# DeepRec-AI/HybridBackend

Measured on AMD Instinct MI355X. Metric: M-lookups/sec, 26-col Criteo-shape dim16, 1/2/4/8 GPUs; % HBM roofline, higher is better.
Workload: dtype f32

## Files before the change

### hybridbackend_amd/_lib.py

```python
import ctypes as C
import os

_HERE = os.path.dirname(os.path.abspath(__file__))
LIB_PATH = os.environ.get('HBK_LIBRARY') or os.path.join(_HERE, 'lib', 'libhbk_core.so')

INT8, UINT8, INT32, UINT32, INT64, UINT64, HALF, FLOAT, DOUBLE = range(9)
APPLY_SGD, APPLY_ADAGRAD = 0, 2
APPLY_LAZY_ADAM, APPLY_FTRL, APPLY_ROWWISE_ADAGRAD = 3, 4, 5
GRAD_DETERMINISTIC = 1
COMBINER_SUM, COMBINER_MEAN, COMBINER_SQRTN = 0, 1, 2
OK, INVALID_ARGUMENT, UNIMPLEMENTED, INTERNAL = 0, 3, 12, 13
COMM_ID_BYTES = 128


class HbkError(RuntimeError):

  def __init__(self, code, message):
    super().__init__(f'[hbk status {code}] {message}')
    self.code = code


class InvalidArgumentError(HbkError, ValueError):
  pass

# ... 325 lines not shown
    'hbk_comm_rccl_versions': (C.c_int, [vp, vp]),
    'hbk_comm_create': (C.c_int, [vp, vp, i32, i32, i32]),
    'hbk_comm_destroy': (C.c_int, [vp]),
    'hbk_comm_check_async': (C.c_int, [vp]),
    'hbk_comm_world_size': (C.c_int, [vp]),
    'hbk_comm_rank': (C.c_int, [vp]),
    'hbk_comm_stream': (vp, [vp]),
    'hbk_comm_active_ranks': (C.c_int, [vp, i32, vp]),
    'hbk_alltoall_n': (C.c_int, [vp, i32, i32, i32, vp, vp, vp, vp]),
    'hbk_alltoallv_wire_workspace_bytes': (sz, [i32, vp, vp, vp, i32]),
    'hbk_alltoallv_n':
      (C.c_int, [vp, i32, i32, i32, i32, vp, vp, vp, vp, vp, vp, sz, vp]),
    'hbk_allreduce_workspace_bytes': (sz, [i32, vp, i32]),
    'hbk_allreduce_n': (C.c_int, [vp, i32, i32, i32, vp, vp, vp, C.c_float, vp, sz, vp]),
    'hbk_allgatherv': (C.c_int, [vp, i32, vp, vp, vp, vp]),
    'hbk_comm_create_custom': (C.c_int, [vp, vp, i32, i32, i32]),
    'hbk_sharded_layout': (C.c_int, [i32, i32] + [vp] * 12),
    'hbk_sharded_create': (C.c_int, [vp, vp, i32, vp, i32]),
    'hbk_sharded_destroy': (C.c_int, [vp]),
    'hbk_sharded_set_hot_rows': (C.c_int, [vp, vp]),
    'hbk_sharded_set_max_norms': (C.c_int, [vp, vp]),
    'hbk_sharded_set_hash_tables': (C.c_int, [vp, vp]),
    'hbk_sharded_lookup_fwd': (C.c_int, [vp, vp, vp, vp, vp, vp, vp, vp]),
    'hbk_sharded_lookup_fwd_weighted': (C.c_int, [vp, vp, vp, vp, vp, vp, vp, vp, vp]),
    'hbk_sharded_prefetch_on': (C.c_int, [vp, vp, vp, vp]),
    'hbk_sharded_lookup_fwd_begin': (C.c_int, [vp, vp, vp, vp, vp, vp]),
    'hbk_sharded_lookup_fwd_end': (C.c_int, [vp, vp, vp, vp]),
    'hbk_sharded_lookup_fwd_ids': (C.c_int, [vp, vp, vp, vp, vp, vp]),
    'hbk_sharded_lookup_fwd_gather': (C.c_int, [vp, vp]),
    'hbk_sharded_hash_missing': (C.c_int, [vp, vp, vp, vp, vp, vp]),
    'hbk_sharded_prefetch': (C.c_int, [vp, vp, vp, vp]),
    'hbk_sharded_owned_ids': (i64, [vp, i32]),
    'hbk_sharded_last_host_us': (C.c_int, [vp, vp]),
    'hbk_sharded_lookup_bwd': (C.c_int, [vp, vp, vp, C.c_float, vp, vp, vp, vp]),
    'hbk_sharded_lookup_bwd_apply': (C.c_int, [vp, vp, vp, i32, C.c_float, vp, vp, vp, vp]),
    'hbk_sharded_set_adam_slots': (C.c_int, [vp, vp, vp]),
    'hbk_sharded_lookup_bwd_adam': (C.c_int, [vp, vp, vp, vp, C.c_float, vp, vp, vp, vp]),
    'hbk_sharded_set_ftrl_slots': (C.c_int, [vp, vp, vp]),
    'hbk_sharded_lookup_bwd_ftrl': (C.c_int, [vp, vp, vp, vp, C.c_float, vp, vp, vp, vp]),
    'hbk_sharded_set_rowwise_adagrad_slots': (C.c_int, [vp, vp]),
    'hbk_sharded_lookup_bwd_rowwise_adagrad': (C.c_int, [vp, vp, vp, vp, C.c_float, vp, vp, vp, vp]),
    'hbk_sharded_lookup_bwd_weights': (C.c_int, [vp, vp, vp, vp, vp]),
  }
  for name, (res, args) in protos.items():
    fn = getattr(l, name)
    fn.restype = res
    fn.argtypes = args


def lib():
  global _lib
  if _lib is not None:
    return _lib
  if not os.path.exists(LIB_PATH):
    raise ImportError(
      f'{LIB_PATH} not found: the gfx950 HIP extension is not built. '
      'Run `python -c "import __graft_entry__ as g; g.build()"` or '
      '`make -C hybridbackend_amd/csrc`. There is no CPU fallback.')
  import torch
  l = C.CDLL(LIB_PATH, mode=C.RTLD_GLOBAL)
  _declare(l)
  _lib = l
  return l


_testing = None
# ... 142 lines not shown
```

### hybridbackend_amd/csrc/common.h

```cpp
#ifndef HBK_CSRC_COMMON_H_
#define HBK_CSRC_COMMON_H_

#include <hip/hip_runtime.h>
#include <stdarg.h>
#include <stdint.h>
#include <stdio.h>

#include "hbk.h"

namespace hbk {

int fail(int code, const char* fmt, ...);

#define HBK_HIP_OK(expr)                                                         \
  do {                                                                           \
    hipError_t e__ = (expr);                                                     \
    if (e__ != hipSuccess) {                                                     \
      return ::hbk::fail(HBK_INTERNAL, "%s failed: %s (%s:%d)", #expr,           \
                         hipGetErrorString(e__), __FILE__, __LINE__);            \
    }                                                                            \
  } while (0)

#define HBK_REQUIRE(cond, ...)                                                   \
  do {                                                                           \
// ... 94 lines not shown
  int bwd_split_pairs = 0;
  int bwd_onepass = 1;
  int fwd_xcd = 1;
  int bwd_xcd = 1;
  int bwd_wide = 1;
  int bwd_group_cols = 0;
  int bwd_dense = 1;
  int bwd_scatter_staged = 1;
  int bwd_rowsort_pos = 64;
  int bwd_pairs_packed = 1;
  int bwd_seg_inline = 1;
  int bwd_scale_fused = 1;
  int bwd_deterministic = 0;
  int bwd_simple = 1;
  int bwd_streams = 4;
  int bwd_lds_pad = 0;
  int bwd_trace = 0;
  int bwd_large_first = 0;
  int bwd_rowsort_ratio = 8;
  int bwd_weights_lds = 1;
  int fwd_d16 = 1;
  int fwd_interleave = 2;
  int fwd_hot_rows = 0;
  int unique_buckets_log2 = -1;
  int partition_sub_tiles = 1;
  int partition_fixed_max = 8;
  int partition_onepass = 1;
  int unique_onepass = 1;
  int sharded_groups = 0;
  int sharded_id64 = 0;
  int sharded_copy_self = 0;
  int sharded_trace = 0;
  int sharded_pack_early = 1;
  int sharded_wire_fused = 1;
  int sharded_inline = 1;
  int sharded_p2p = 1;
  int sharded_p2p_test_refuse = -1;
  int sync_wait_ms = 2000;
  int sync_onepass_off = 0;
  int sync_test_withhold = -1;
};
Options& options();

struct SyncTake {
  int32_t* words;
  int32_t* zero;
  int64_t zero_words;
  int32_t* status;
  int32_t* summary;
  int32_t* poison;
  unsigned long long wait_ticks;
  int32_t withhold;
};
struct SyncWait {
  int32_t* status;
  int32_t* summary;
  int32_t* poison;
  unsigned long long ticks;
  int32_t withhold;
  int32_t pad_;
};
inline SyncWait sync_wait_of(const SyncTake& t) {
  SyncWait w;
  w.status = t.status;
  w.summary = t.summary;
  w.poison = t.poison;
// ... 89 lines not shown
```

### hybridbackend_amd/csrc/misc.cpp

```cpp
#include <stdlib.h>
#include <string.h>

#include <vector>

#include "common.h"

namespace hbk {
namespace {
thread_local char g_last_error[1024] = "";
}

int fail(int code, const char* fmt, ...) {
  va_list ap;
  va_start(ap, fmt);
  vsnprintf(g_last_error, sizeof(g_last_error), fmt, ap);
  va_end(ap);
  return code;
}
}

namespace hbk {
namespace {
struct OptionEntry {
  const char* name;
// ... 10 lines not shown
    {"bwd_scatter_staged", "HBK_BWD_SCATTER_STAGED", &Options::bwd_scatter_staged},
    {"bwd_rowsort_pos", "HBK_BWD_ROWSORT_POS", &Options::bwd_rowsort_pos},
    {"bwd_rowsort_ratio", "HBK_BWD_ROWSORT_RATIO", &Options::bwd_rowsort_ratio},
    {"bwd_deterministic", "HBK_BWD_DETERMINISTIC", &Options::bwd_deterministic},
    {"bwd_streams", "HBK_BWD_STREAMS", &Options::bwd_streams},
    {"bwd_trace", "HBK_BWD_TRACE", &Options::bwd_trace},
    {"bwd_lds_pad", "HBK_BWD_LDS_PAD", &Options::bwd_lds_pad},
    {"bwd_large_first", "HBK_BWD_LARGE_FIRST", &Options::bwd_large_first},
    {"bwd_pairs_packed", "HBK_BWD_PAIRS_PACKED", &Options::bwd_pairs_packed},
    {"bwd_seg_inline", "HBK_BWD_SEG_INLINE", &Options::bwd_seg_inline},
    {"bwd_scale_fused", "HBK_BWD_SCALE_FUSED", &Options::bwd_scale_fused},
    {"bwd_simple", "HBK_BWD_SIMPLE", &Options::bwd_simple},
    {"fwd_d16", "HBK_FWD_D16", &Options::fwd_d16},
    {"bwd_weights_lds", "HBK_BWD_WEIGHTS_LDS", &Options::bwd_weights_lds},
    {"bwd_wide", "HBK_BWD_WIDE", &Options::bwd_wide},
    {"bwd_xcd", "HBK_BWD_XCD", &Options::bwd_xcd},
    {"fwd_xcd", "HBK_FWD_XCD", &Options::fwd_xcd},
    {"fwd_hot_rows", "HBK_FWD_HOT", &Options::fwd_hot_rows},
    {"fwd_interleave", "HBK_FWD_INTERLEAVE", &Options::fwd_interleave},
    {"unique_buckets_log2", "HBK_UNIQUE_LOG2P", &Options::unique_buckets_log2},
    {"partition_sub_tiles", "HBK_PART_SUB", &Options::partition_sub_tiles},
    {"partition_fixed_max", "HBK_PART_FIXED", &Options::partition_fixed_max},
    {"partition_onepass", "HBK_PART_ONEPASS", &Options::partition_onepass},
    {"unique_onepass", "HBK_UNIQUE_ONEPASS", &Options::unique_onepass},
    {"sharded_groups", "HBK_SHARDED_GROUPS", &Options::sharded_groups},
    {"sharded_id64", "HBK_SHARDED_ID64", &Options::sharded_id64},
    {"sharded_copy_self", "HBK_SHARDED_COPY_SELF", &Options::sharded_copy_self},
    {"sharded_trace", "HBK_SHARDED_TRACE", &Options::sharded_trace},
    {"sharded_inline", "HBK_SHARDED_INLINE", &Options::sharded_inline},
    {"sharded_p2p", "HBK_SHARDED_P2P", &Options::sharded_p2p},
    {"sharded_p2p_test_refuse", "HBK_SHARDED_P2P_TEST_REFUSE", &Options::sharded_p2p_test_refuse},
    {"sharded_wire_fused", "HBK_SHARDED_WIRE_FUSED", &Options::sharded_wire_fused},
    {"sharded_pack_early", "HBK_SHARDED_PACK_EARLY", &Options::sharded_pack_early},
    {"sync_wait_ms", "HBK_SYNC_WAIT_MS", &Options::sync_wait_ms},
    {"sync_onepass_off", "HBK_SYNC_ONEPASS_OFF", &Options::sync_onepass_off},
    {"sync_test_withhold", "HBK_SYNC_TEST_WITHHOLD", &Options::sync_test_withhold},
};

Options from_environment() {
  Options o;
  for (const OptionEntry& e : kOptions) {
    const char* v = getenv(e.env);
    if (v != nullptr && *v != 0) o.*(e.field) = atoi(v);
  }
  return o;
}
}

Options& options() {
  static Options o = from_environment();
  return o;
}
}

extern "C" const char* hbk_last_error(void) { return hbk::g_last_error; }

extern "C" int hbk_set_option(const char* name, int32_t value) {
  using namespace hbk;
  HBK_REQUIRE(name != nullptr, "set_option: name is NULL");
  for (const OptionEntry& e : kOptions) {
    if (strcmp(e.name, name) == 0) {
      options().*(e.field) = value;
      return HBK_OK;
    }
  }
  return fail(HBK_INVALID_ARGUMENT, "set_option: unknown option '%s'", name);
// ... 117 lines not shown
```

### hybridbackend_amd/csrc/sharded.hip

```cpp
#include <stdio.h>
#include <stdlib.h>
#include <string.h>
#include <unistd.h>

#include <algorithm>
#include <chrono>
#include <functional>
#include <random>
#include <utility>
#include <vector>

#include "common.h"

namespace hbk {
int alltoallv_events(hbk_comm_t comm, int32_t n, int32_t dtype, int32_t wire_dtype,
                     int32_t topology, const int64_t* common_sizes, const void* const* inputs,
                     const int32_t* send_sizes, void* const* outputs,
                     const int32_t* recv_sizes, void* wire_ws, size_t wire_ws_bytes,
                     hbk_stream_t compute_stream, hipEvent_t before, hipEvent_t after,
                     bool skip_self, bool inline_x);
int partition_by_modulo_fused(int32_t n_cols, int32_t num_partitions, const int64_t* const* inputs,
                              const int64_t* lens, const int64_t* buckets,
                              int64_t* const* outputs, int32_t* const* sizes,
                              int32_t* const* indices, int32_t* sizes_t, void* workspace,
                              size_t workspace_bytes, hipStream_t stream);
namespace {

constexpr int kBlock = 256;
constexpr int kMaxSegs = 480;
constexpr int kMaxPackWorldP2p = 256;
constexpr int kCopyTileBytes = kBlock * 16 * 8;

struct Seg {
  const void* src;
  void* dst;
  int64_t bytes;
  int32_t tile0;
  int32_t narrow;
};

struct SegArgs {
  int32_t n_segs;
  int32_t pad_;
  Seg seg[kMaxSegs];
};
// ... 195 lines not shown
      } else {
        qh = mid;
      }
    }
    const int64_t at = base[q] + (e - cum[q]);
    if (at < 0 || at >= a.dst_items) continue;
    if (a.narrow) {
      reinterpret_cast<int32_t*>(a.dst)[at] = (int32_t)v;
    } else {
      reinterpret_cast<int64_t*>(a.dst)[at] = v;
    }
  }
  if (a.slots == nullptr) return;
  const int32_t* idx = a.idx[c];
#pragma unroll
  for (int k = 0; k < kPackTile / kBlock; ++k) {
    const int32_t j = e0 + k * kBlock + tid;
    if (j >= n) break;
    const int32_t e = __builtin_nontemporal_load(idx + j);
    if (e < 0 || e >= cum[W]) continue;
    int q = 0, qh = W;
    while (qh - q > 1) {
      const int mid = (q + qh) >> 1;
      if (cum[mid] <= e) {
        q = mid;
      } else {
        qh = mid;
      }
    }
    const int64_t at = base[q] + (e - cum[q]);
    if (at < 0 || at >= a.dst_items) continue;
    a.slots[at] = j;
  }
}

constexpr int kDedupTile = 2048;

struct DedupArgs {
  const int64_t* uniq;
  const int32_t* inv;
  int32_t* idx;
  const int32_t* nu;
  int32_t* S;
  int32_t* St;
  FastDiv wdiv;
  int32_t n_cols, W, N, pad_;
  int64_t off[kMaxPackCols];
  int32_t n[kMaxPackCols];
  int32_t tile0[kMaxPackCols];
  int16_t col[kMaxPackCols];
};
static_assert(sizeof(DedupArgs) <= 16384, "kernarg budget");

__global__ __launch_bounds__(kBlock) void dedup_compose_kernel(const DedupArgs a) {
  int d = 0, hi = a.n_cols;
  while (hi - d > 1) {
    const int mid = (d + hi) >> 1;
    if (a.tile0[mid] <= (int)blockIdx.x) {
      d = mid;
    } else {
      hi = mid;
    }
  }
  const int32_t n = a.n[d];
  const int32_t* inv = a.inv + a.off[d];
  int32_t* idx = a.idx + a.off[d];
// ... 161 lines not shown
  bool trace;
  int n_groups;
  bool inline_x;
  std::vector<hbk_sharded_column_t> cols;
  std::vector<int64_t> n_ids, n_seg;
  std::vector<int64_t> n_sent;
  std::vector<const int32_t*> row_splits;
  hbk::SlotPair adam;
  hbk::SlotPair ftrl;
  hbk::SlotPair rowwise;
  std::vector<float> max_norms;
  std::vector<int32_t> lowp;
  bool lowp_wire16 = false;
  std::vector<hbk_sharded_hash_t> hash;
  bool any_hash = false;
  hbk::Buffer slots_buf;
  std::vector<const float*> id_weights;
  std::vector<int32_t> send_sizes;
  std::vector<int32_t> recv_sizes;
  std::vector<hbk::Group> groups;
  std::vector<int64_t> fwd_own_id_off;
  hipEvent_t ev[4][4];
  bool have_step;
  bool rows_live = false;
  float host_us[3];
  hbk::Buffer part_ws, ids_buf, rows_buf, wire_ws, bwd_ws, runs_dev;
  char* send_ids_p;
  char* recv_ids_p;
  float* send_rows_p;
  float* recv_rows_p;
  bool any_dedup;
  hbk::Buffer dedup_tmp;
  bool pack_early;
  bool fused_half;
  bool zero_copy_grads;
  bool zero_copy_self;
  struct PartSet {
    hbk::Buffer part_out, shard_index, sizes_dev;
    hbk::Buffer uniq, inv, nu, uniq_ws;
    hbk::Buffer packed;
    bool packed_early = false;
    hbk::Buffer slots;
    bool has_slots = false;
    int32_t* host_sizes = nullptr;
    hipEvent_t done = nullptr;
    hipEvent_t ready = nullptr;
    std::vector<const int64_t*> ids;
    std::vector<int64_t> n_ids;
    bool pending = false;
  } ps[2];
  int cur;
  hipStream_t pre_stream;
  hipEvent_t step_begin;
  bool prefetch_used;
  bool fwd_open = false;
  bool ids_open = false;
  bool fin_wire = false, fin_hop = false, fin_p2p = false;
  bool fin_prefetched = false;
  int32_t* fin_slot_send = nullptr;
  hbk::Buffer missing_ws;
  int fin_use = 0;
  std::chrono::steady_clock::time_point fin_t0;
  float fin_us[2] = {0.f, 0.f};
  bool p2p_opt = false;
  bool p2p_bound = false;
  std::vector<float*> p2p_outs;
// ... 12 lines not shown
  HBK_REQUIRE(plan != nullptr && comm != nullptr, "sharded_create: NULL argument");
  HBK_REQUIRE(n_cols >= 1 && cols != nullptr, "sharded_create: need at least one column");
  HBK_REQUIRE(wire_dtype == HBK_FLOAT || wire_dtype == HBK_HALF,
              "sharded_create: wire_dtype must be float or half");
  for (int32_t c = 0; c < n_cols; ++c) {
    HBK_REQUIRE(cols[c].dim >= 1 && cols[c].rows_local >= 0 && cols[c].bucket >= 0,
                "sharded_create: column %d: bad dim / rows / bucket", c);
    HBK_REQUIRE(cols[c].combiner >= HBK_COMBINER_SUM && cols[c].combiner <= HBK_COMBINER_SQRTN,
                "sharded_create: column %d: unknown combiner %d", c, cols[c].combiner);
    HBK_REQUIRE(cols[c].shard != nullptr || cols[c].rows_local == 0,
                "sharded_create: column %d: shard is NULL", c);
  }
  hbk_sharded* p = new hbk_sharded();
  p->comm = comm;
  p->W = hbk_comm_world_size(comm);
  p->rank = hbk_comm_rank(comm);
  p->N = n_cols;
  p->wire_dtype = wire_dtype;
  p->cols.assign(cols, cols + n_cols);
  p->max_norms.assign((size_t)n_cols, 0.0f);
  p->id32 = options().sharded_id64 == 0;
  p->trace = options().sharded_trace != 0;
  p->n_groups = options().sharded_groups;
  p->inline_x = options().sharded_inline != 0;
  p->p2p_opt = options().sharded_p2p != 0;
  for (int32_t c = 0; c < n_cols; ++c) {
    if (cols[c].bucket <= 0 || cols[c].bucket > 0x7fffffffll) p->id32 = false;
  }
  p->have_step = false;
  p->any_dedup = false;
  for (int32_t c = 0; c < n_cols; ++c) p->any_dedup = p->any_dedup || cols[c].dedup != 0;
  p->fused_half = wire_dtype == HBK_HALF && options().sharded_wire_fused != 0;
  p->pack_early = options().sharded_pack_early != 0;
  p->zero_copy_self = (wire_dtype == HBK_FLOAT || p->fused_half) && options().sharded_copy_self == 0;
  p->zero_copy_grads = p->zero_copy_self && wire_dtype == HBK_FLOAT;
  p->send_ids_p = p->recv_ids_p = nullptr;
  p->send_rows_p = p->recv_rows_p = nullptr;
  p->cur = 0;
  p->pre_stream = nullptr;
  p->step_begin = nullptr;
  p->prefetch_used = false;
  p->host_runs = nullptr;
  for (auto& st : p->ev) {
    for (auto& e : st) {
      if (hipEventCreateWithFlags(&e, hipEventDisableTiming) != hipSuccess) {
        delete p;
        return fail(HBK_INTERNAL, "sharded_create: hipEventCreate failed");
      }
    }
  }
  bool ok = hipEventCreateWithFlags(&p->step_begin, hipEventDisableTiming) == hipSuccess;
  for (auto& set : p->ps) {
    ok = ok && hipEventCreateWithFlags(&set.done, hipEventDisableTiming) == hipSuccess &&
         hipEventCreateWithFlags(&set.ready, hipEventDisableTiming) == hipSuccess &&
         hipHostMalloc(reinterpret_cast<void**>(&set.host_sizes),
                       sizeof(int32_t) * 3 * (size_t)n_cols * p->W,
                       hipHostMallocDefault) == hipSuccess;
  }
  if (!ok ||
      hipHostMalloc(reinterpret_cast<void**>(&p->host_runs),
                    sizeof(int64_t) * 7 * (size_t)n_cols * p->W, hipHostMallocDefault) !=
          hipSuccess) {
    hbk_sharded_destroy(p);
    return fail(HBK_INTERNAL, "sharded_create: could not create streams / events / pinned memory");
  }
  *plan = p;
// ... 54 lines not shown
  s.narrow = narrow;
  return s;
}

int exchange(hbk_sharded* p, int32_t dtype, int32_t wire, const void* in, const int32_t* send,
             void* out, const int32_t* recv, hbk_stream_t stream, hipEvent_t before = nullptr,
             hipEvent_t after = nullptr, void* wire_ws = nullptr, size_t wire_ws_bytes = 0,
             bool skip_self = false) {
  const int64_t cs[1] = {1};
  const void* vin[1] = {in};
  void* vout[1] = {out};
  if (wire != dtype && wire_ws == nullptr) {
    const size_t wws = hbk_alltoallv_wire_workspace_bytes(1, cs, send, recv, p->W);
    int rc = p->wire_ws.ensure(wws + 16);
    if (rc != HBK_OK) return rc;
    wire_ws = p->wire_ws.ptr;
    wire_ws_bytes = p->wire_ws.bytes;
  }
  return alltoallv_events(p->comm, 1, dtype, wire, HBK_TOPOLOGY_ALL, cs, vin, send, vout, recv,
                          wire_ws, wire_ws_bytes, stream, before, after, skip_self,
                          p->inline_x && before != nullptr);
}

int pipeline_groups(int n_cols, int world, int requested) {
  int g = requested >= 1 && requested <= 4 ? requested : 2;
  if (world == 1 && !(requested >= 1 && requested <= 4)) g = 1;
  return g < n_cols ? g : n_cols;
}

int step_groups(const hbk_sharded* p) {
  if (p->p2p_bound) return 1;
  return p->inline_x && !(p->n_groups >= 1 && p->n_groups <= 4)
             ? 1 : pipeline_groups(p->N, p->W, p->n_groups);
}

int run_partition(hbk_sharded* p, hbk_sharded::PartSet& set, const int64_t* const* ids,
                  const int64_t* n_ids, hipStream_t stream) {
  const int N = p->N, W = p->W;
  int64_t total = 0;
  for (int c = 0; c < N; ++c) {
    HBK_REQUIRE(n_ids[c] >= 0 && n_ids[c] < (1ll << 31), "sharded lookup: bad n_ids[%d]", c);
    total += n_ids[c];
  }
  int rc;
  if ((rc = set.part_out.ensure((size_t)total * 8 + 8)) != HBK_OK) return rc;
  if ((rc = set.shard_index.ensure((size_t)total * 4 + 8)) != HBK_OK) return rc;
  if ((rc = set.sizes_dev.ensure((size_t)N * W * 4 * 3)) != HBK_OK) return rc;
  if ((rc = set.packed.ensure((size_t)total * (p->id32 ? 4 : 8) + 16)) != HBK_OK) return rc;
  std::vector<int64_t*> pout(N);
  std::vector<int32_t*> sizes(N), idx(N);
  std::vector<int64_t> buckets(N);
  int32_t* sizes_dev = reinterpret_cast<int32_t*>(set.sizes_dev.ptr);
  int32_t* sizes_t = sizes_dev + (size_t)N * W;
  int32_t* recv_t = sizes_t + (size_t)N * W;
  int64_t off = 0;
  for (int c = 0; c < N; ++c) {
    pout[c] = reinterpret_cast<int64_t*>(set.part_out.ptr) + off;
    idx[c] = reinterpret_cast<int32_t*>(set.shard_index.ptr) + off;
    sizes[c] = sizes_dev + (size_t)c * W;
    buckets[c] = p->cols[c].bucket;
    off += n_ids[c];
  }
  const size_t ws = hbk_partition_workspace_bytes(N, n_ids, W);
  if ((rc = p->part_ws.ensure(ws + 8)) != HBK_OK) return rc;
  rc = partition_by_modulo_fused(N, W, ids, n_ids, buckets.data(), pout.data(), sizes.data(),
                                 idx.data(), sizes_t, p->part_ws.ptr, p->part_ws.bytes, stream);
// ... 40 lines not shown
                        set.uniq_ws.ptr, set.uniq_ws.bytes, reinterpret_cast<hbk_stream_t>(stream));
      if (rc != HBK_OK) return rc;
      a.uniq = reinterpret_cast<const int64_t*>(set.uniq.ptr);
      a.inv = reinterpret_cast<const int32_t*>(set.inv.ptr);
      a.idx = reinterpret_cast<int32_t*>(set.shard_index.ptr);
      a.nu = reinterpret_cast<const int32_t*>(set.nu.ptr);
      a.S = sizes_dev;
      a.St = sizes_t;
      a.wdiv = make_fastdiv((uint64_t)W);
      a.wdiv.d = (uint64_t)W;
      a.n_cols = nd;
      a.W = W;
      a.N = N;
      a.pad_ = 0;
      hipLaunchKernelGGL(dedup_compose_kernel, dim3((unsigned)tiles), dim3(kBlock), 0, stream, a);
      hipLaunchKernelGGL(dedup_sizes_kernel, dim3((unsigned)nd), dim3(kMaxPackWorld), 0, stream, a);
      HBK_HIP_OK(hipGetLastError());
    }
  }
  const void* sin[1] = {sizes_t};
  void* sout[1] = {recv_t};
  const int64_t cnt[1] = {(int64_t)N * W};
  rc = hbk_alltoall_n(p->comm, 1, HBK_INT32, HBK_TOPOLOGY_ALL, sin, cnt, sout,
                      reinterpret_cast<hbk_stream_t>(stream));
  if (rc != HBK_OK) return rc;
  HBK_HIP_OK(hipMemcpyAsync(set.host_sizes, sizes_dev, sizeof(int32_t) * 3 * N * W,
                            hipMemcpyDeviceToHost, stream));
  HBK_HIP_OK(hipEventRecord(set.done, stream));
  set.packed_early = p->pack_early && N <= kMaxPackCols && W <= kMaxPackWorld && total > 0;
  set.has_slots = false;
  if (set.packed_early) {
    PackArgs a;
    a.slots = nullptr;
    if (p->p2p_bound) {
      if ((rc = set.slots.ensure((size_t)total * 4 + 16)) != HBK_OK) return rc;
      a.slots = reinterpret_cast<int32_t*>(set.slots.ptr);
      set.has_slots = true;
    }
    a.S = sizes_dev;
    a.dst = set.packed.ptr;
    a.dst_items = total;
    a.n_cols = N;
    a.W = W;
    a.narrow = p->id32 ? 1 : 0;
    a.pad_ = 0;
    const int G = step_groups(p);
    int64_t tiles = 0, gbase = 0;
    for (int g = 0; g < G; ++g) {
      const int c0 = (int)((int64_t)N * g / G), c1 = (int)((int64_t)N * (g + 1) / G);
      int64_t in_group = 0;
      for (int c = c0; c < c1; ++c) {
        a.src[c] = id_src[c];
        a.idx[c] = idx[c];
        a.gbase[c] = gbase;
        a.n[c] = (int32_t)n_ids[c];
        a.tile0[c] = (int32_t)tiles;
        a.g0[c] = (int16_t)c0;
        a.g1[c] = (int16_t)c1;
        tiles += (n_ids[c] + kPackTile - 1) / kPackTile;
        in_group += n_ids[c];
      }
      gbase += in_group;
    }
    hipLaunchKernelGGL(pack_ids_kernel, dim3((unsigned)tiles), dim3(kBlock), 0, stream, a);
    HBK_HIP_OK(hipGetLastError());
  }
  HBK_HIP_OK(hipEventRecord(set.ready, stream));
// ... 577 lines not shown
      }
      c0 += k;
    }
  }
  const bool wire = !(W == 1 && zc);
  const bool hop = wire && !p->inline_x;
  if (hop) HBK_HIP_OK(hipEventRecord(p->ev[0][0], stream));
  for (int g = 0; g < G && wire; ++g) {
    const Group& gr = groups[g];
    rc = exchange(p, id_dtype, id_dtype, ids_send_base + gr.id_send * id_bytes,
                  gr.lay.ids_send_peer.data(), ids_recv_base + gr.id_recv * id_bytes,
                  gr.lay.ids_recv_peer.data(), stream_, p->ev[0][0], p->ev[1][g], nullptr, 0, zc);
    if (rc != HBK_OK) return rc;
    if (p2p) {
      rc = exchange(p, HBK_INT32, HBK_INT32, slot_send + gr.id_send, gr.lay.ids_send_peer.data(),
                    slot_recv + gr.id_recv, gr.lay.ids_recv_peer.data(), stream_, p->ev[0][0],
                    p->ev[3][0], nullptr, 0, zc);
      if (rc != HBK_OK) return rc;
    }
  }
  p->fin_wire = wire;
  p->fin_hop = hop;
  p->fin_p2p = p2p;
  p->fin_use = use;
  p->fin_t0 = t_begin;
  p->fin_us[0] = (float)t_enq1;
  p->fin_us[1] = (float)(t_sync - t_enq1);
  p->fin_prefetched = prefetched;
  p->fin_slot_send = slot_send;
  p->ids_open = true;
  return HBK_OK;
}

int fwd_gather(hbk_sharded_t p, hbk_stream_t stream_) {
  p->ids_open = false;
  hipStream_t stream = as_stream(stream_);
  const int N = p->N, W = p->W, me = p->rank;
  const bool wire = p->fin_wire, hop = p->fin_hop, p2p = p->fin_p2p;
  const bool zc = p->zero_copy_self, half = p->fused_half, any_hash = p->any_hash;
  const bool lowp = !p->lowp.empty(), wire16 = p->lowp_wire16;
  const int32_t id_dtype = p->id32 ? HBK_INT32 : HBK_INT64;
  const std::vector<Group>& groups = p->groups;
  const int G = (int)groups.size();
  int64_t* const slots_base = reinterpret_cast<int64_t*>(p->slots_buf.ptr);
  int32_t* const slot_send = p->fin_slot_send;
  int32_t* const slot_recv = reinterpret_cast<int32_t*>(p->slot_recv.ptr);
  float* const rows_send_base = p->send_rows_p;
  float* const rows_recv_base = p->recv_rows_p;
  int rc;
  for (int g = 0; g < G; ++g) {
    const Group& gr = groups[g];
    const int ng = gr.c1 - gr.c0;
    if (hop) HBK_HIP_OK(hipStreamWaitEvent(stream, p->ev[1][g], 0));
    if (hop && p2p) HBK_HIP_OK(hipStreamWaitEvent(stream, p->ev[3][0], 0));
    auto run_ids = [&](int q, int c) { return received_ids_at(p, gr, q, c); };
    if (any_hash && (rc = translate_group(p, gr, run_ids, slots_base, stream_)) != HBK_OK) return rc;
    std::vector<hbk_lookup_column_t> v;
    std::vector<float> clip;
    std::vector<int32_t> lowp_dtype;
    v.reserve((size_t)ng * W);
    for (int q = 0; q < W; ++q) {
      for (int c = 0; c < ng; ++c) {
        const int64_t n = gr.R[(size_t)q * ng + c];
        if (n == 0) continue;
        clip.push_back(p->max_norms[(size_t)(gr.c0 + c)]);
        if (lowp) lowp_dtype.push_back(p->lowp[(size_t)(gr.c0 + c)]);
        const hbk_sharded_column_t& col = p->cols[gr.c0 + c];
        hbk_lookup_column_t h;
        memset(&h, 0, sizeof(h));
        h.table = col.shard;
        h.rows = col.rows_local;
        h.dim = col.dim;
        h.ids_dtype = id_dtype;
        h.n_ids = n;
        h.n_segments = n;
        h.divisor = W;
        h.combiner = HBK_COMBINER_SUM;
        h.hot_rows = col.hot_rows;
        int64_t out_at = gr.row_send + gr.lay.own_row_off[(size_t)q * ng + c];
        float* out_base = rows_send_base;
        h.ids = run_ids(q, c);
        if (any_hash && p->hash[(size_t)(gr.c0 + c)].keys_cache != nullptr) {
          h.ids_dtype = HBK_INT64;
          h.ids = slots_base + gr.id_recv + gr.lay.own_id_off[(size_t)q * ng + c];
          h.divisor = 1;
        }
        if (zc && q == me) {
          out_at = gr.row_recv + gr.lay.req_row_off[(size_t)q * ng + c];
          out_base = rows_recv_base;
        }
        if (p2p) {
          h.out = p->peer_out[(size_t)q * N + gr.c0 + c];
          h.out_stride = p->peer_stride[(size_t)q * N + gr.c0 + c];
          h.out_slots = slot_recv + gr.id_recv + gr.lay.own_id_off[(size_t)q * ng + c];
          if (zc && q == me) {
            h.out_slots = slot_send + gr.id_send + gr.lay.req_id_off[(size_t)q * ng + c];
          }
          h.hot_rows = 0;
        } else if (half || wire16) {
          h.out = reinterpret_cast<float*>(reinterpret_cast<uint16_t*>(out_base) + out_at);
          h.half_io = half ? HBK_LOOKUP_OUT_HALF : 0;
        } else {
          h.out = out_base + out_at;
        }
        v.push_back(h);
      }
    }
    if (lowp) {
      if (wire16) {
        std::vector<hbk_lowp_gather_column_t> lv(v.size());
        for (size_t i = 0; i < v.size(); ++i) {
          const hbk_lookup_column_t& h = v[i];
          hbk_lowp_gather_column_t& d = lv[i];
          memset(&d, 0, sizeof(d));
          d.table = h.table;
          d.dim = h.dim;
          d.ids_dtype = h.ids_dtype;
          d.rows = h.rows;
          d.ids = h.ids;
          d.n_ids = h.n_ids;
          d.divisor = h.divisor;
          d.out = h.out;
        }
        rc = hbk_lowp_gather_rows_n((int32_t)lv.size(), lv.data(), stream_);
      } else {
        std::vector<hbk_lowp_lookup_column_t> lv(v.size());
        for (size_t i = 0; i < v.size(); ++i) {
          const hbk_lookup_column_t& h = v[i];
          hbk_lowp_lookup_column_t& d = lv[i];
          memset(&d, 0, sizeof(d));
          d.table = h.table;
// ... 159 lines not shown
      HBK_REQUIRE(outs[c] == p->p2p_outs[c] &&
                      (out_strides == nullptr || out_strides[c] == 0 ||
                       out_strides[c] == p->p2p_strides[c] ||
                       (out_strides[c] == p->cols[c].dim && p->p2p_strides[c] == p->cols[c].dim)),
                  "sharded_lookup_fwd: column %d: not the output registered with "
                  "hbk_sharded_p2p_bind", c);
    }
  }
  for (int g = 0; g < G && wire && !p2p; ++g) {
    const Group& gr = groups[g];
    if (half || wire16) {
      rc = exchange(p, HBK_HALF, HBK_HALF, reinterpret_cast<uint16_t*>(rows_send_base) + gr.row_send,
                    gr.lay.rows_send_peer.data(),
                    reinterpret_cast<uint16_t*>(rows_recv_base) + gr.row_recv,
                    gr.lay.rows_recv_peer.data(), stream_, p->ev[2][g], p->ev[3][g], nullptr, 0, zc);
    } else {
      rc = exchange(p, HBK_FLOAT, p->wire_dtype, rows_send_base + gr.row_send,
                    gr.lay.rows_send_peer.data(), rows_recv_base + gr.row_recv,
                    gr.lay.rows_recv_peer.data(), stream_, p->ev[2][g], p->ev[3][g],
                    p->wire_ws.ptr, p->wire_ws.bytes, zc);
    }
    if (rc != HBK_OK) return rc;
  }
  std::vector<int32_t*> idx((size_t)N);
  {
    int64_t off = 0;
    for (int c = 0; c < N; ++c) {
      idx[c] = reinterpret_cast<int32_t*>(set.shard_index.ptr) + off;
      off += n_ids[c];
    }
  }
  const int64_t* d_start = reinterpret_cast<const int64_t*>(p->runs_dev.ptr);
  const int64_t* d_base = d_start + (size_t)N * W;
  for (int g = 0; g < G && !p2p; ++g) {
    const Group& gr = groups[g];
    const int ng = gr.c1 - gr.c0;
    if (hop) HBK_HIP_OK(hipStreamWaitEvent(stream, p->ev[3][g], 0));
    std::vector<hbk_lookup_column_t> v(ng);
    for (int c = 0; c < ng; ++c) {
      const int cc = gr.c0 + c;
      hbk_lookup_column_t& h = v[c];
      memset(&h, 0, sizeof(h));
      h.table = half || wire16 ? reinterpret_cast<const float*>(reinterpret_cast<const uint16_t*>(rows_recv_base) +
                                                                gr.row_recv)
                               : rows_recv_base + gr.row_recv;
      h.half_io = half ? HBK_LOOKUP_TABLE_HALF : 0;
      h.rows = p->n_sent[cc];
      h.dim = p->cols[cc].dim;
      h.ids_dtype = HBK_INT32;
      h.ids = idx[cc];
      h.n_ids = n_ids[cc];
      h.row_splits = p->row_splits[cc];
      h.n_segments = p->n_seg[cc];
      h.divisor = 1;
      h.combiner = p->cols[cc].combiner;
      h.out = outs[cc];
      h.out_stride = out_strides ? out_strides[cc] : 0;
      h.run_start = d_start + (size_t)cc * W;
      h.run_base = d_base + (size_t)cc * W;
      h.n_runs = W;
      h.id_weights = p->id_weights[cc];
    }
    if (wire16) {
      std::vector<hbk_lowp_lookup_runs_column_t> lv((size_t)ng);
      for (int c = 0; c < ng; ++c) {
        const hbk_lookup_column_t& h = v[c];
        hbk_lowp_lookup_runs_column_t& d = lv[(size_t)c];
        memset(&d, 0, sizeof(d));
        d.col.table = h.table;
        d.col.table_dtype = p->lowp[(size_t)(gr.c0 + c)];
        d.col.dim = h.dim;
        d.col.rows = h.rows;
        d.col.ids = h.ids;
        d.col.ids_dtype = h.ids_dtype;
        d.col.combiner = h.combiner;
        d.col.n_ids = h.n_ids;
        d.col.row_splits = h.row_splits;
        d.col.n_segments = h.n_segments;
        d.col.divisor = 1;
        d.col.out_stride = h.out_stride;
        d.col.out = h.out;
        d.col.id_weights = h.id_weights;
        d.run_start = h.run_start;
        d.run_base = h.run_base;
        d.n_runs = h.n_runs;
      }
      rc = hbk_lowp_lookup_fwd_runs(ng, lv.data(), stream_);
    } else {
      rc = hbk_group_lookup_fwd(ng, v.data(), stream_);
    }
    if (rc != HBK_OK) return rc;
  }
  p->have_step = true;
  p->rows_live = !p2p;
  const double total = std::chrono::duration<double, std::micro>(std::chrono::steady_clock::now() -
                                                                p->fin_t0).count();
  p->host_us[0] = p->fin_us[0];
  p->host_us[1] = p->fin_us[1];
  p->host_us[2] = (float)(total - p->fin_us[0] - p->fin_us[1]);
  return HBK_OK;
}

extern "C" int hbk_sharded_lookup_fwd(hbk_sharded_t p, const int64_t* const* ids,
                                      const int64_t* n_ids,
                                      const int32_t* const* row_splits,
                                      const int64_t* n_segments, float* const* outs,
                                      const int32_t* out_strides, hbk_stream_t stream_) {
  using namespace hbk;
  HBK_REQUIRE(outs != nullptr, "sharded_lookup_fwd: NULL argument array");
  const int rc = hbk_sharded_lookup_fwd_begin(p, ids, n_ids, row_splits, n_segments, stream_);
  if (rc != HBK_OK) return rc;
  return hbk_sharded_lookup_fwd_end(p, outs, out_strides, stream_);
}

extern "C" int hbk_sharded_lookup_fwd_weighted(hbk_sharded_t p, const int64_t* const* ids,
                                               const int64_t* n_ids,
                                               const int32_t* const* row_splits,
                                               const int64_t* n_segments,
                                               const float* const* id_weights, float* const* outs,
                                               const int32_t* out_strides, hbk_stream_t stream_) {
  using namespace hbk;
  HBK_REQUIRE(p != nullptr && outs != nullptr, "sharded_lookup_fwd: NULL argument");
  bool weighted = false;
  for (int c = 0; id_weights != nullptr && c < p->N; ++c) weighted = weighted || id_weights[c] != nullptr;
  for (int c = 0; weighted && c < p->N; ++c) {
    HBK_REQUIRE(id_weights[c] == nullptr || p->cols[c].bucket > 0,
                "sharded_lookup_fwd_weighted: column %d: id_weights need a bucket (hbk_sharded_column_t."
                "bucket > 0) so that every id names a row of its owner's shard", c);
  }
  if (weighted && p->p2p_bound) {
    return fail(HBK_UNIMPLEMENTED, "sharded_lookup_fwd_weighted: the p2p form (hbk_sharded_p2p_bind) has "
                "no stitch to apply id_weights in");
  }
  int rc = hbk_sharded_lookup_fwd_begin(p, ids, n_ids, row_splits, n_segments, stream_);
  if (rc != HBK_OK) return rc;
  for (int c = 0; weighted && c < p->N; ++c) p->id_weights[c] = id_weights[c];
  return hbk_sharded_lookup_fwd_end(p, outs, out_strides, stream_);
}

extern "C" int hbk_sharded_prefetch_on(hbk_sharded_t p, const int64_t* const* ids,
                                       const int64_t* n_ids, hbk_stream_t stream_) {
  using namespace hbk;
  HBK_REQUIRE(p != nullptr && ids && n_ids, "sharded_prefetch_on: NULL argument");
  hbk_sharded::PartSet& set = p->ps[p->cur ^ 1];
// ... 515 lines not shown
    return fail(HBK_UNIMPLEMENTED, "%s: the plan has a hash column (hbk_sharded_set_hash_tables): its rows are fp32",
                who);
  }
  if (p->p2p_bound) {
    return fail(HBK_UNIMPLEMENTED, "%s: the plan is p2p-bound (hbk_sharded_p2p_bind): the p2p form's owner gather "
                "stores fp32 rows", who);
  }
  p->adam = SlotPair();
  p->ftrl = SlotPair();
  p->rowwise = SlotPair();
  p->lowp.assign(dtypes, dtypes + p->N);
  p->lowp_wire16 = wire == HBK_LOWP_WIRE_TABLE;
  p->have_step = false;
  p->rows_live = false;
  p->fwd_open = p->ids_open = false;
  return HBK_OK;
}

extern "C" int hbk_sharded_set_hot_rows(hbk_sharded_t p, const int32_t* hot_rows) {
  using namespace hbk;
  HBK_REQUIRE(p != nullptr && hot_rows != nullptr, "sharded_set_hot_rows: NULL argument");
  for (int c = 0; c < p->N; ++c) p->cols[c].hot_rows = hot_rows[c] != 0 ? 1 : 0;
  return HBK_OK;
}

extern "C" int hbk_sharded_last_host_us(hbk_sharded_t p, float* out3) {
  using namespace hbk;
  HBK_REQUIRE(p != nullptr && out3 != nullptr, "sharded_last_host_us: NULL argument");
  HBK_REQUIRE(p->have_step, "sharded_last_host_us: no forward step yet");
  for (int i = 0; i < 3; ++i) out3[i] = p->host_us[i];
  return HBK_OK;
}

extern "C" int64_t hbk_sharded_owned_ids(hbk_sharded_t p, int32_t column) {
  if (p == nullptr || !(p->have_step || p->ids_open || p->fwd_open) || column < 0 || column >= p->N) return -1;
  int64_t n = 0;
  for (int q = 0; q < p->W; ++q) n += p->recv_sizes[(size_t)q * p->N + column];
  return n;
}
```

### hybridbackend_amd/embedding/sharded.py

```python
import ctypes as C
import threading

import torch

from hybridbackend_amd import _lib
from hybridbackend_amd import _marshal
from hybridbackend_amd.distribute import partition as _partition
from hybridbackend_amd.embedding.lookup import GroupLookup
from hybridbackend_amd.embedding.lookup import GroupLookupGrad
from hybridbackend_amd.embedding import optimizer as _opt


class _Step:
  __slots__ = ('ids', 'row_splits', 'send_ids', 'send_sizes', 'shard_index', 'send_sizes_host',
               'recv_sizes_host', 'recv_ids', 'send_rows', 'recv_rows', 'outs')

  def __init__(self):
    for s in self.__slots__:
      setattr(self, s, None)


_PLAN_LOCK = threading.RLock()


# ... 84 lines not shown
    from hybridbackend_amd.embedding.lookup import _combiner_code
    n = len(self.shards)
    combs = self.combiners
    if isinstance(combs, (str, int)) or combs is None:
      combs = [combs] * n
    cols = (_lib.ShardedColumn * n)()
    for c, t in enumerate(self.shards):
      cols[c].shard = t.data_ptr()
      cols[c].rows_local = t.shape[0]
      cols[c].dim = t.shape[1]
      cols[c].combiner = _combiner_code(combs[c])
      cols[c].bucket = self.buckets[c]
      cols[c].hot_rows = 1 if self.hot_rows[c] else 0
      cols[c].dedup = 1 if self.dedup[c] else 0
      if self.accums is not None:
        cols[c].accum = self.accums[c].data_ptr()
    self._plan_handle = C.c_void_p()
    wire = _lib.HALF if self.wire_dtype == torch.float16 else _lib.FLOAT
    _lib.check(self._lib.hbk_sharded_create(
      C.byref(self._plan_handle), self.coll._handle, n, cols, wire))
    self._plan_created()
    if any(self.max_norms):
      _lib.check(self._lib.hbk_sharded_set_max_norms(self._plan_handle, (C.c_float * n)(*self.max_norms)))
    for opt, slots in _opt.bound(self):
      opt.set_sharded_slots(self._plan_handle, slots)

  def _plan_created(self):
    """Hook: plan state a subclass sets right after creation (ShardedHashGroupLookup: its tables)."""

  def last_host_us(self):
    out = (C.c_float * 3)()
    _lib.check(self._lib.hbk_sharded_last_host_us(self._plan(), out))
    return tuple(float(v) for v in out)

  def p2p_bind(self, outs):
    n = len(self.shards)
    if len(outs) != n:
      raise _lib.InvalidArgumentError(_lib.INVALID_ARGUMENT, f'p2p_bind: {len(outs)} outputs for {n} columns')
    for c, o in enumerate(outs):
      _lib.require_device_tensor(o, 'output', row_strided=True)
      if o.dtype != torch.float32 or o.dim() != 2 or o.shape[1] != self.dims[c]:
        raise _lib.InvalidArgumentError(_lib.INVALID_ARGUMENT, f'p2p_bind: output {c} must be fp32 [*, {self.dims[c]}]')
    strides = (C.c_int32 * n)(*[0 if o.is_contiguous() else int(o.stride(0)) for o in outs])
    rows = _lib.i64_array([int(o.shape[0]) for o in outs])
    rc = self._lib.hbk_sharded_p2p_bind(self._plan(), _lib.ptr_array([o.data_ptr() for o in outs]),
                                        strides, rows, _lib.current_stream(self.device))
    if rc == _lib.UNIMPLEMENTED:
      self._p2p_keep = None
      return False
    _lib.check(rc)
    self._p2p_keep = list(outs)
    return True

  def p2p_unbind(self):
    _lib.check(self._lib.hbk_sharded_p2p_unbind(self._plan()))
    self._p2p_keep = None

  def close(self):
    if getattr(self, '_plan_handle', None) is not None:
      self._lib.hbk_sharded_destroy(self._plan_handle)
      self._plan_handle = None

  def bind(self, ids, row_splits=None, outs=None, sp_weights=None):
    bound = self._bind(ids, row_splits, outs)
    if sp_weights is not None and any(w is not None for w in sp_weights):
      from hybridbackend_amd import _marshal
# ... 391 lines not shown
```

### include/hbk.h

```cpp
#ifndef HBK_H_
#define HBK_H_

#include <stddef.h>
#include <stdint.h>

#ifdef __cplusplus
extern "C" {
#endif

typedef void* hbk_stream_t;

#define HBK_OK 0
#define HBK_INVALID_ARGUMENT 3
#define HBK_UNIMPLEMENTED 12
#define HBK_INTERNAL 13

#define HBK_INT8 0
#define HBK_UINT8 1
#define HBK_INT32 2
#define HBK_UINT32 3
#define HBK_INT64 4
#define HBK_UINT64 5
#define HBK_HALF 6
#define HBK_FLOAT 7
// ... 678 lines not shown
} hbk_sharded_hash_t;
int hbk_sharded_set_hash_tables(hbk_sharded_t plan, const hbk_sharded_hash_t* tables );
int hbk_sharded_destroy(hbk_sharded_t plan);
int hbk_sharded_lookup_fwd(hbk_sharded_t plan, const int64_t* const* ids, const int64_t* n_ids,
                           const int32_t* const* row_splits, const int64_t* n_segments,
                           float* const* outs, const int32_t* out_strides, hbk_stream_t stream);
int hbk_sharded_lookup_fwd_weighted(hbk_sharded_t plan, const int64_t* const* ids,
                                    const int64_t* n_ids, const int32_t* const* row_splits,
                                    const int64_t* n_segments, const float* const* id_weights,
                                    float* const* outs, const int32_t* out_strides,
                                    hbk_stream_t stream);
int hbk_sharded_lookup_fwd_begin(hbk_sharded_t plan, const int64_t* const* ids,
                                 const int64_t* n_ids, const int32_t* const* row_splits,
                                 const int64_t* n_segments, hbk_stream_t stream);
int hbk_sharded_lookup_fwd_end(hbk_sharded_t plan, float* const* outs, const int32_t* out_strides,
                               hbk_stream_t stream);
int hbk_sharded_lookup_fwd_ids(hbk_sharded_t plan, const int64_t* const* ids, const int64_t* n_ids,
                               const int32_t* const* row_splits, const int64_t* n_segments,
                               hbk_stream_t stream);
int hbk_sharded_lookup_fwd_gather(hbk_sharded_t plan, hbk_stream_t stream);
int hbk_sharded_hash_missing(hbk_sharded_t plan, const uint8_t* want , int64_t* const* out_ids,
                             const int64_t* out_capacity, int64_t* counts ,
                             hbk_stream_t stream);
int hbk_sharded_prefetch(hbk_sharded_t plan, const int64_t* const* ids, const int64_t* n_ids,
                         void* ids_ready_event );
int hbk_sharded_prefetch_on(hbk_sharded_t plan, const int64_t* const* ids, const int64_t* n_ids,
                            hbk_stream_t stream);
int64_t hbk_sharded_owned_ids(hbk_sharded_t plan, int32_t column);

int hbk_sharded_p2p_bind(hbk_sharded_t plan, float* const* outs, const int32_t* out_strides,
                         const int64_t* out_rows, hbk_stream_t stream);
int hbk_sharded_p2p_unbind(hbk_sharded_t plan);
int hbk_sharded_last_host_us(hbk_sharded_t plan, float* out3);
int hbk_sharded_lookup_bwd_weights(hbk_sharded_t plan, const float* const* grads,
                                   const int32_t* grad_strides, float* const* grad_weights,
                                   hbk_stream_t stream);
int hbk_sharded_lookup_bwd(hbk_sharded_t plan, const float* const* grads,
                           const int32_t* grad_strides, float apply_lr,
                           int64_t* const* unique_rows, float* const* grad_rows,
                           int32_t* const* n_unique, hbk_stream_t stream);
int hbk_sharded_lookup_bwd_apply(hbk_sharded_t plan, const float* const* grads,
                                 const int32_t* grad_strides, int32_t apply, float apply_lr,
                                 int64_t* const* unique_rows, float* const* grad_rows,
                                 int32_t* const* n_unique, hbk_stream_t stream);
int hbk_sharded_set_adam_slots(hbk_sharded_t plan, float* const* m, float* const* v);
int hbk_sharded_lookup_bwd_adam(hbk_sharded_t plan, const float* const* grads,
                                const int32_t* grad_strides, const hbk_adam_t* adam, float lr,
                                int64_t* const* unique_rows, float* const* grad_rows,
                                int32_t* const* n_unique, hbk_stream_t stream);
int hbk_sharded_set_ftrl_slots(hbk_sharded_t plan, float* const* accum, float* const* linear);
int hbk_sharded_lookup_bwd_ftrl(hbk_sharded_t plan, const float* const* grads,
                                const int32_t* grad_strides, const hbk_ftrl_t* ftrl, float lr,
                                int64_t* const* unique_rows, float* const* grad_rows,
                                int32_t* const* n_unique, hbk_stream_t stream);
int hbk_sharded_set_rowwise_adagrad_slots(hbk_sharded_t plan, float* const* accum);
int hbk_sharded_lookup_bwd_rowwise_adagrad(hbk_sharded_t plan, const float* const* grads,
                                           const int32_t* grad_strides,
                                           const hbk_rowwise_adagrad_t* rowwise_adagrad, float lr,
                                           int64_t* const* unique_rows, float* const* grad_rows,
                                           int32_t* const* n_unique, hbk_stream_t stream);

#ifdef __cplusplus
}
#endif
#endif
```

Before: 29970.

## Write local lookups directly to outputs and scatter received rows by slot

For simple float-wire sharded forward lookups at small world sizes, the local shard writes gathered rows straight into the caller's output tensors using the pack slot map. It skips the intermediate receive buffer and the reassembly pass. Rows received from peers go through a new multi-run scatter kernel that places them at their slot positions, replacing the per-column run-based gather. This removes one round of HBM traffic for self-owned rows, at the cost of writing slots during packing, extra host-side eligibility checks, and a new kernel launch path.

```diff
diff --git a/hybridbackend_amd/_lib.py b/hybridbackend_amd/_lib.py
--- a/hybridbackend_amd/_lib.py
+++ b/hybridbackend_amd/_lib.py
@@ -381,6 +381,7 @@
     'hbk_sharded_prefetch': (C.c_int, [vp, vp, vp, vp]),
     'hbk_sharded_owned_ids': (i64, [vp, i32]),
     'hbk_sharded_last_host_us': (C.c_int, [vp, vp]),
+    'hbk_sharded_last_form': (C.c_int, [vp, vp]),
     'hbk_sharded_lookup_bwd': (C.c_int, [vp, vp, vp, C.c_float, vp, vp, vp, vp]),
     'hbk_sharded_lookup_bwd_apply': (C.c_int, [vp, vp, vp, i32, C.c_float, vp, vp, vp, vp]),
     'hbk_sharded_set_adam_slots': (C.c_int, [vp, vp, vp]),
diff --git a/hybridbackend_amd/csrc/common.h b/hybridbackend_amd/csrc/common.h
--- a/hybridbackend_amd/csrc/common.h
+++ b/hybridbackend_amd/csrc/common.h
@@ -150,6 +150,7 @@
   int sharded_copy_self = 0;
   int sharded_trace = 0;
   int sharded_pack_early = 1;
+  int sharded_direct = 1;
   int sharded_wire_fused = 1;
   int sharded_inline = 1;
   int sharded_p2p = 1;
diff --git a/hybridbackend_amd/csrc/misc.cpp b/hybridbackend_amd/csrc/misc.cpp
--- a/hybridbackend_amd/csrc/misc.cpp
+++ b/hybridbackend_amd/csrc/misc.cpp
@@ -66,6 +66,7 @@
     {"sharded_p2p_test_refuse", "HBK_SHARDED_P2P_TEST_REFUSE", &Options::sharded_p2p_test_refuse},
     {"sharded_wire_fused", "HBK_SHARDED_WIRE_FUSED", &Options::sharded_wire_fused},
     {"sharded_pack_early", "HBK_SHARDED_PACK_EARLY", &Options::sharded_pack_early},
+    {"sharded_direct", "HBK_SHARDED_DIRECT", &Options::sharded_direct},
     {"sync_wait_ms", "HBK_SYNC_WAIT_MS", &Options::sync_wait_ms},
     {"sync_onepass_off", "HBK_SYNC_ONEPASS_OFF", &Options::sync_onepass_off},
     {"sync_test_withhold", "HBK_SYNC_TEST_WITHHOLD", &Options::sync_test_withhold},
diff --git a/hybridbackend_amd/csrc/sharded.hip b/hybridbackend_amd/csrc/sharded.hip
--- a/hybridbackend_amd/csrc/sharded.hip
+++ b/hybridbackend_amd/csrc/sharded.hip
@@ -10,7 +10,7 @@
 #include <utility>
 #include <vector>
 
-#include "common.h"
+#include "lookup_common.h"
 
 namespace hbk {
 int alltoallv_events(hbk_comm_t comm, int32_t n, int32_t dtype, int32_t wire_dtype,
@@ -272,6 +272,114 @@
     if (at < 0 || at >= a.dst_items) continue;
     a.slots[at] = j;
   }
+}
+
+constexpr int kScatterRuns = 128;
+constexpr int kScatterU = 4;
+constexpr int kScatterWaves = kBlock / kWave;
+
+struct ScatterRun {
+  const float* src;
+  float* out;
+  const int32_t* slots;
+  int32_t n;
+  int32_t n_rows;
+  int32_t dim;
+  int32_t out_stride;
+  int32_t chunks;
+  int32_t lpr_log2;
+};
+
+struct ScatterArgs {
+  int32_t n_runs;
+  int32_t pad_;
+  int32_t tile_start[kScatterRuns + 1];
+  ScatterRun run[kScatterRuns];
+};
+static_assert(sizeof(ScatterArgs) <= 16384, "kernarg budget");
+
+template <typename V>
+__global__ __launch_bounds__(kBlock) void scatter_rows_kernel(const ScatterArgs a) {
+  constexpr int VE = sizeof(V) / 4;
+  const int b = (int)blockIdx.x;
+  const int lane = lane_id();
+  const int nr = a.n_runs;
+  const int t0 = lane < nr ? a.tile_start[lane] : 0x7fffffff;
+  const int t1 = lane + kWave < nr ? a.tile_start[lane + kWave] : 0x7fffffff;
+  int ri = (int)__builtin_popcountll(__ballot(t0 <= b)) + (int)__builtin_popcountll(__ballot(t1 <= b)) - 1;
+  ri = __builtin_amdgcn_readfirstlane(ri);
+  const ScatterRun& r = a.run[ri];
+  const int wave = (int)(threadIdx.x >> 6);
+  const int lpr_log2 = r.lpr_log2;
+  const int rpi = kWave >> lpr_log2;
+  const int sub = lane & ((1 << lpr_log2) - 1);
+  const int grp = lane >> lpr_log2;
+  const int32_t n = r.n;
+  const int64_t row0 = ((int64_t)(b - a.tile_start[ri]) * kScatterWaves + wave) * (int64_t)(kScatterU * rpi);
+  if (row0 >= n) return;
+  int32_t slotreg[kScatterU];
+#pragma unroll
+  for (int k = 0; k < kScatterU; ++k) {
+    const int q = k * kWave + lane;
+    slotreg[k] = -1;
+    if (q < kScatterU * rpi && row0 + q < n) slotreg[k] = __builtin_nontemporal_load(r.slots + row0 + q);
+  }
+  const bool live = sub < r.chunks;
+  V v[kScatterU];
+#pragma unroll
+  for (int u = 0; u < kScatterU; ++u) {
+    const int64_t j = row0 + u * rpi + grp;
+    v[u] = zero_v<V>();
+    if (live && j < n) {
+      v[u] = __builtin_nontemporal_load(reinterpret_cast<const V*>(r.src + j * (int64_t)r.dim + (int64_t)sub * VE));
+    }
+  }
+#pragma unroll
+  for (int u = 0; u < kScatterU; ++u) {
+    const int q0 = u * rpi;
+    const int k = q0 >> 6;
+    int32_t s = slotreg[0];
+#pragma unroll
+    for (int kk = 1; kk < kScatterU; ++kk) s = (k == kk) ? slotreg[kk] : s;
+    const int32_t dst = __shfl(s, (q0 & (kWave - 1)) + grp, kWave);
+    const int64_t j = row0 + q0 + grp;
+    if (live && j < n && (uint32_t)dst < (uint32_t)r.n_rows) {
+      __builtin_nontemporal_store(
+          v[u], reinterpret_cast<V*>(r.out + (int64_t)dst * (int64_t)r.out_stride + (int64_t)sub * VE));
+    }
+  }
+}
+
+int scatter_runs(const std::vector<ScatterRun>& runs, const std::vector<uint8_t>& vec4, hipStream_t stream) {
+  for (int wide = 0; wide < 2; ++wide) {
+    size_t i = 0;
+    while (i < runs.size()) {
+      ScatterArgs args;
+      int k = 0;
+      int64_t tiles = 0;
+      args.tile_start[0] = 0;
+      while (i < runs.size() && k < kScatterRuns) {
+        const size_t at = i++;
+        if ((int)vec4[at] != wide || runs[at].n <= 0) continue;
+        args.run[k] = runs[at];
+        const int64_t per_block = (int64_t)kScatterWaves * kScatterU * (kWave >> runs[at].lpr_log2);
+        tiles += (runs[at].n + per_block - 1) / per_block;
+        HBK_REQUIRE(tiles < (1ll << 31), "sharded_lookup_fwd: scatter grid too large");
+        ++k;
+        args.tile_start[k] = (int32_t)tiles;
+      }
+      if (k == 0) continue;
+      args.n_runs = k;
+      args.pad_ = 0;
+      if (wide) {
+        hipLaunchKernelGGL(scatter_rows_kernel<f32x4>, dim3((unsigned)tiles), dim3(kBlock), 0, stream, args);
+      } else {
+        hipLaunchKernelGGL(scatter_rows_kernel<float>, dim3((unsigned)tiles), dim3(kBlock), 0, stream, args);
+      }
+      HBK_HIP_OK(hipGetLastError());
+    }
+  }
+  return HBK_OK;
 }
 
 constexpr int kDedupTile = 2048;
@@ -499,6 +607,9 @@
   bool any_dedup;
   hbk::Buffer dedup_tmp;
   bool pack_early;
+  int direct_opt;
+  std::vector<uint8_t> direct_col;
+  int32_t last_form[2] = {0, 0};
   bool fused_half;
   bool zero_copy_grads;
   bool zero_copy_self;
@@ -577,6 +688,7 @@
   for (int32_t c = 0; c < n_cols; ++c) p->any_dedup = p->any_dedup || cols[c].dedup != 0;
   p->fused_half = wire_dtype == HBK_HALF && options().sharded_wire_fused != 0;
   p->pack_early = options().sharded_pack_early != 0;
+  p->direct_opt = options().sharded_direct;
   p->zero_copy_self = (wire_dtype == HBK_FLOAT || p->fused_half) && options().sharded_copy_self == 0;
   p->zero_copy_grads = p->zero_copy_self && wire_dtype == HBK_FLOAT;
   p->send_ids_p = p->recv_ids_p = nullptr;
@@ -697,6 +809,12 @@
   if (p->p2p_bound) return 1;
   return p->inline_x && !(p->n_groups >= 1 && p->n_groups <= 4)
              ? 1 : pipeline_groups(p->N, p->W, p->n_groups);
+}
+
+constexpr int kDirectMaxWorld = 2;
+bool may_produce_slots(const hbk_sharded* p) {
+  return p->direct_opt != 0 && (p->direct_opt >= 2 || p->W <= kDirectMaxWorld) && p->wire_dtype == HBK_FLOAT && p->zero_copy_self && p->lowp.empty() && !p->any_hash &&
+         !p->any_dedup && !p->p2p_bound && p->pack_early;
 }
 
 int run_partition(hbk_sharded* p, hbk_sharded::PartSet& set, const int64_t* const* ids,
@@ -803,7 +921,7 @@
   if (set.packed_early) {
     PackArgs a;
     a.slots = nullptr;
-    if (p->p2p_bound) {
+    if (p->p2p_bound || may_produce_slots(p)) {
       if ((rc = set.slots.ensure((size_t)total * 4 + 16)) != HBK_OK) return rc;
       a.slots = reinterpret_cast<int32_t*>(set.slots.ptr);
       set.has_slots = true;
@@ -1447,11 +1565,25 @@
   return HBK_OK;
 }
 
-int fwd_gather(hbk_sharded_t p, hbk_stream_t stream_) {
+int fwd_gather(hbk_sharded_t p, hbk_stream_t stream_, float* const* outs = nullptr,
+               const int32_t* out_strides = nullptr) {
   p->ids_open = false;
   hipStream_t stream = as_stream(stream_);
   const int N = p->N, W = p->W, me = p->rank;
   const bool wire = p->fin_wire, hop = p->fin_hop, p2p = p->fin_p2p;
+  p->direct_col.assign((size_t)N, 0);
+  const hbk_sharded::PartSet& set = p->ps[p->fin_use];
+  const int32_t* const own_slots = reinterpret_cast<const int32_t*>(set.slots.ptr);
+  if (outs != nullptr && !p2p && may_produce_slots(p) && set.packed_early && set.has_slots && own_slots != nullptr) {
+    for (int c = 0; c < N; ++c) {
+      RowShape shape;
+      const int32_t stride = out_strides != nullptr ? out_strides[c] : 0;
+      p->direct_col[(size_t)c] =
+          p->row_splits[c] == nullptr && p->id_weights[c] == nullptr && p->max_norms[(size_t)c] == 0.0f &&
+          p->cols[c].hot_rows == 0 && (outs[c] != nullptr || p->n_ids[c] == 0) && (stride == 0 || stride >= p->cols[c].dim) &&
+          make_rowshape(p->cols[c].dim, (uintptr_t)outs[c] | ((uintptr_t)(uint32_t)stride * 4), &shape);
+    }
+  }
   const bool zc = p->zero_copy_self, half = p->fused_half, any_hash = p->any_hash;
   const bool lowp = !p->lowp.empty(), wire16 = p->lowp_wire16;
   const int32_t id_dtype = p->id32 ? HBK_INT32 : HBK_INT64;
@@ -1512,6 +1644,11 @@
             h.out_slots = slot_send + gr.id_send + gr.lay.req_id_off[(size_t)q * ng + c];
           }
           h.hot_rows = 0;
+        } else if (q == me && p->direct_col[(size_t)(gr.c0 + c)] != 0) {
+          h.out = outs[gr.c0 + c];
+          h.out_stride = out_strides != nullptr ? out_strides[gr.c0 + c] : 0;
+          h.out_slots = own_slots + gr.id_send + gr.lay.req_id_off[(size_t)q * ng + c];
+          h.hot_rows = 0;
         } else if (half || wire16) {
           h.out = reinterpret_cast<float*>(reinterpret_cast<uint16_t*>(out_base) + out_at);
           h.half_io = half ? HBK_LOOKUP_OUT_HALF : 0;
@@ -1737,10 +1874,16 @@
   }
   const int64_t* d_start = reinterpret_cast<const int64_t*>(p->runs_dev.ptr);
   const int64_t* d_base = d_start + (size_t)N * W;
+  p->direct_col.resize((size_t)N, 0);
+  const std::vector<uint8_t>& direct = p->direct_col;
+  const int32_t* const own_slots = reinterpret_cast<const int32_t*>(set.slots.ptr);
+  const int me = p->rank;
+  int32_t n_direct = 0, n_scattered = 0;
   for (int g = 0; g < G && !p2p; ++g) {
     const Group& gr = groups[g];
     const int ng = gr.c1 - gr.c0;
     if (hop) HBK_HIP_OK(hipStreamWaitEvent(stream, p->ev[3][g], 0));
+    int direct_here = 0;
     std::vector<hbk_lookup_column_t> v(ng);
     for (int c = 0; c < ng; ++c) {
       const int cc = gr.c0 + c;
@@ -1765,6 +1908,41 @@
       h.run_base = d_base + (size_t)cc * W;
       h.n_runs = W;
       h.id_weights = p->id_weights[cc];
+      if (direct[(size_t)cc] != 0) {
+        h.n_ids = h.n_segments = 0;
+        ++n_direct;
+        ++direct_here;
+      }
+    }
+    if (direct_here > 0) {
+      std::vector<ScatterRun> runs;
+      std::vector<uint8_t> vec4;
+      for (int q = 0; q < W; ++q) {
+        for (int c = 0; c < ng && q != me; ++c) {
+          const int cc = gr.c0 + c;
+          const int64_t n = p->send_sizes[(size_t)cc * W + q];
+          if (direct[(size_t)cc] == 0 || n <= 0) continue;
+          ScatterRun r;
+          r.src = rows_recv_base + gr.row_recv + gr.lay.req_row_off[(size_t)q * ng + c];
+          r.out = outs[cc];
+          r.slots = own_slots + gr.id_send + gr.lay.req_id_off[(size_t)q * ng + c];
+          r.n = (int32_t)n;
+          r.n_rows = (int32_t)p->n_seg[cc];
+          r.dim = p->cols[cc].dim;
+          r.out_stride = out_strides != nullptr && out_strides[cc] > 0 ? out_strides[cc] : r.dim;
+          RowShape shape;
+          HBK_REQUIRE(make_rowshape(r.dim, (uintptr_t)r.src | (uintptr_t)r.out | ((uintptr_t)(uint32_t)r.out_stride * 4),
+                                    &shape),
+                      "sharded_lookup_fwd: column %d: dim %d needs more than 64 lanes per row", cc, r.dim);
+          r.chunks = shape.chunks;
+          r.lpr_log2 = shape.lpr_log2;
+          runs.push_back(r);
+          vec4.push_back(shape.vec4);
+        }
+      }
+      n_scattered += (int32_t)runs.size();
+      if (!runs.empty() && (rc = scatter_runs(runs, vec4, stream)) != HBK_OK) return rc;
+      if (direct_here == ng) continue;
     }
     if (wire16) {
       std::vector<hbk_lowp_lookup_runs_column_t> lv((size_t)ng);
@@ -1798,6 +1976,8 @@
   }
   p->have_step = true;
   p->rows_live = !p2p;
+  p->last_form[0] = n_direct;
+  p->last_form[1] = n_scattered;
   const double total = std::chrono::duration<double, std::micro>(std::chrono::steady_clock::now() -
                                                                 p->fin_t0).count();
   p->host_us[0] = p->fin_us[0];
@@ -1813,8 +1993,9 @@
                                       const int32_t* out_strides, hbk_stream_t stream_) {
   using namespace hbk;
   HBK_REQUIRE(outs != nullptr, "sharded_lookup_fwd: NULL argument array");
-  const int rc = hbk_sharded_lookup_fwd_begin(p, ids, n_ids, row_splits, n_segments, stream_);
+  int rc = fwd_ids(p, ids, n_ids, row_splits, n_segments, stream_);
   if (rc != HBK_OK) return rc;
+  if ((rc = fwd_gather(p, stream_, outs, out_strides)) != HBK_OK) return rc;
   return hbk_sharded_lookup_fwd_end(p, outs, out_strides, stream_);
 }
 
@@ -2396,6 +2577,15 @@
   return HBK_OK;
 }
 
+extern "C" int hbk_sharded_last_form(hbk_sharded_t p, int32_t out[2]) {
+  using namespace hbk;
+  HBK_REQUIRE(p != nullptr && out != nullptr, "sharded_last_form: NULL argument");
+  HBK_REQUIRE(p->have_step, "sharded_last_form: no forward step yet");
+  out[0] = p->last_form[0];
+  out[1] = p->last_form[1];
+  return HBK_OK;
+}
+
 extern "C" int64_t hbk_sharded_owned_ids(hbk_sharded_t p, int32_t column) {
   if (p == nullptr || !(p->have_step || p->ids_open || p->fwd_open) || column < 0 || column >= p->N) return -1;
   int64_t n = 0;
diff --git a/hybridbackend_amd/embedding/sharded.py b/hybridbackend_amd/embedding/sharded.py
--- a/hybridbackend_amd/embedding/sharded.py
+++ b/hybridbackend_amd/embedding/sharded.py
@@ -140,6 +140,11 @@
     out = (C.c_float * 3)()
     _lib.check(self._lib.hbk_sharded_last_host_us(self._plan(), out))
     return tuple(float(v) for v in out)
+
+  def last_form(self):
+    out = (C.c_int32 * 2)()
+    _lib.check(self._lib.hbk_sharded_last_form(self._plan(), out))
+    return int(out[0]), int(out[1])
 
   def p2p_bind(self, outs):
     n = len(self.shards)
diff --git a/include/hbk.h b/include/hbk.h
--- a/include/hbk.h
+++ b/include/hbk.h
@@ -734,6 +734,7 @@
                          const int64_t* out_rows, hbk_stream_t stream);
 int hbk_sharded_p2p_unbind(hbk_sharded_t plan);
 int hbk_sharded_last_host_us(hbk_sharded_t plan, float* out3);
+int hbk_sharded_last_form(hbk_sharded_t plan, int32_t out[2]);
 int hbk_sharded_lookup_bwd_weights(hbk_sharded_t plan, const float* const* grads,
                                    const int32_t* grad_strides, float* const* grad_weights,
                                    hbk_stream_t stream);
```

Measured after the change: 30080, median of 2. Within noise of the previous version (+0.4%).
